# pityka/lamp

Measured on AMD Instinct MI355X. Metric: training-step samples/sec, higher is better.
Workload: dtype bf16; 1 GPU; example-cifar100 Cnn.resnet(100) training step (fwd+backprop+AdamW), synthetic CIFAR batch; per_gpu_batch=2048, global_batch=2048, parallelism=single, optimizer=AdamW lr 1e-3 wd 0 beta2 0.95 mixedPrecision

## Files before the change

include/lamp_hip.h:

```cpp
#ifndef LAMP_HIP_H
#define LAMP_HIP_H

#include <stddef.h>
#include <stdint.h>

#ifdef __cplusplus
extern "C" {
#endif

#define LAMP_MAX_DIMS 8

typedef struct lamp_tensor lamp_tensor;
typedef struct lamp_stream lamp_stream;
typedef struct lamp_comm lamp_comm;
typedef struct lamp_graph lamp_graph;

#define LAMP_U8 0
#define LAMP_I8 1
#define LAMP_I16 2
#define LAMP_I32 3
#define LAMP_I64 4
#define LAMP_F16 5
#define LAMP_F32 6
#define LAMP_F64 7
#define LAMP_BOOL 11
#define LAMP_BF16 15

#define LAMP_DEVICE_CPU (-1)

const char* lamp_last_error(void);
const char* lamp_version(void);

int lamp_has_gpu(int* out);
int lamp_get_num_gpus(int* out);
int lamp_get_device(int* out);
int lamp_set_device(int device);
int lamp_device_synchronize(void);
int lamp_flush_deferred(void);
int lamp_device_name(char* buf, int buflen);
int lamp_device_num_cus(int* out);
int lamp_stream_get_current(int device, lamp_stream** out);
int lamp_stream_get_default(int device, lamp_stream** out);
int lamp_stream_get_from_pool(int high_priority, int device, lamp_stream** out);
int lamp_stream_set_current(lamp_stream* s);
int lamp_stream_synchronize(lamp_stream* s);
int lamp_stream_wait_stream(lamp_stream* waiter, lamp_stream* on);
int lamp_stream_release(lamp_stream* s);
int lamp_tensor_record_stream(const lamp_tensor* t, lamp_stream* s_or_null);
int lamp_stream_native(lamp_stream* s, void** hip_stream_out);
int lamp_manual_seed(uint64_t seed);
int lamp_allow_tf32(int flag);

int lamp_kernel_timer_enable(int on);
// ... 529 lines not shown
```

jni/LampNative.java:

```java
package aten;

public final class LampNative {
  static { System.loadLibrary("lampjni"); }
  private LampNative() {}
  public static native String lamp_last_error();
  public static native String lamp_version();
  public static native void lamp_tensor_release_all(long[] tensors);
  public static native byte[] lamp_comm_get_unique_id();
  public static native long lamp_comm_init_rank(int nranks, byte[] id, int rank);
  public static native long[] lamp_tensors_from_file(String path, long offset, long length, boolean pin, long[] types, long[] offsets, long[] lengths);
  public static native long[] lamp_tensor_trace_list();
  public static native long[] lamp_tensor_sizes(long t);
  public static native long[] lamp_tensor_strides(long t);
  public static native boolean copyFromDoubleArray(long t, double[] a);
  public static native boolean copyToDoubleArray(long t, double[] a);
  public static native boolean copyFromFloatArray(long t, float[] a);
  public static native boolean copyToFloatArray(long t, float[] a);
  public static native boolean copyFromLongArray(long t, long[] a);
  public static native boolean copyToLongArray(long t, long[] a);
  public static native boolean copyFromIntArray(long t, int[] a);
  public static native boolean copyToIntArray(long t, int[] a);
  public static native boolean copyFromShortArray(long t, short[] a);
  public static native boolean copyToShortArray(long t, short[] a);
  public static native boolean copyFromByteArray(long t, byte[] a);
  public static native boolean copyToByteArray(long t, byte[] a);

  public static native int lamp_has_gpu();
  public static native int lamp_get_num_gpus();
  public static native int lamp_get_device();
  public static native void lamp_set_device(int device);
  public static native void lamp_device_synchronize();
  public static native void lamp_flush_deferred();
  public static native int lamp_device_num_cus();
  public static native long lamp_stream_get_current(int device);
  public static native long lamp_stream_get_default(int device);
  public static native long lamp_stream_get_from_pool(int high_priority, int device);
  public static native void lamp_stream_set_current(long s);
  public static native void lamp_stream_synchronize(long s);
  public static native void lamp_stream_wait_stream(long waiter, long on);
  public static native void lamp_stream_release(long s);
  public static native void lamp_tensor_record_stream(long t, long s_or_null);
  public static native void lamp_manual_seed(long seed);
  public static native void lamp_allow_tf32(int flag);
  public static native void lamp_kernel_timer_enable(int on);
  public static native void lamp_kernel_timer_filter(String tag);
  public static native double lamp_kernel_timer_calibrate();
  public static native void lamp_device_shared_hint(int device, int delta);
// ... 335 lines not shown
```

jni/aten_jni.c:

```c
#ifdef LAMP_JNI_SYNTAX_CHECK
#include "jni_syntax_check.h"
#else
#include <jni.h>
#endif
#include <stdint.h>
#include <stddef.h>
#include "lamp_hip.h"

#define H(x) ((void*)(intptr_t)(x))

#define LAMP_JNI_MAX_OUTS 4096

static void lamp_throw(JNIEnv* env) {
  jclass ex = (*env)->FindClass(env, "java/lang/RuntimeException");
  if (ex) (*env)->ThrowNew(env, ex, lamp_last_error());
}
static void lamp_throw_msg(JNIEnv* env, const char* msg) {
  jclass ex = (*env)->FindClass(env, "java/lang/RuntimeException");
  if (ex) (*env)->ThrowNew(env, ex, msg);
}

#define COPY_NATIVES(JT, JNAME, GET, REL)                                                                                              \
  JNIEXPORT jboolean JNICALL Java_aten_LampNative_copyFrom##JNAME##Array(JNIEnv* env, jclass cls, jlong t, JT##Array a) {              \
    (void)cls;                                                                                                                         \
// ... 120 lines not shown
  (void)cls;
  const int rc_ = lamp_set_device((int)device);
  if (rc_ != 0) { lamp_throw(env); return; }
}

JNIEXPORT void JNICALL Java_aten_LampNative_lamp_1device_1synchronize(JNIEnv* env, jclass cls) {
  (void)cls;
  const int rc_ = lamp_device_synchronize();
  if (rc_ != 0) { lamp_throw(env); return; }
}

JNIEXPORT void JNICALL Java_aten_LampNative_lamp_1flush_1deferred(JNIEnv* env, jclass cls) {
  (void)cls;
  const int rc_ = lamp_flush_deferred();
  if (rc_ != 0) { lamp_throw(env); return; }
}

JNIEXPORT jint JNICALL Java_aten_LampNative_lamp_1device_1num_1cus(JNIEnv* env, jclass cls) {
  (void)cls;
  int out_o = 0;
  const int rc_ = lamp_device_num_cus(&out_o);
  if (rc_ != 0) { lamp_throw(env); return 0; }
  return (jint)out_o;
}

JNIEXPORT jlong JNICALL Java_aten_LampNative_lamp_1stream_1get_1current(JNIEnv* env, jclass cls, jint device) {
  (void)cls;
  void* out_o = NULL;
  const int rc_ = lamp_stream_get_current((int)device, (void*)&out_o);
  if (rc_ != 0) { lamp_throw(env); return 0; }
// ... 3239 lines not shown
```

lamp_amd/csrc/core/runtime.cpp:

```cpp
#include "tensor.h"

#include <unordered_map>
#include <atomic>
#include <mutex>
#include <set>
#include <map>

struct lamp_stream {
  hipStream_t s = nullptr;
  int device = 0;
  bool is_default = false;
  std::atomic<int> refs{1};
};

struct lamp_graph {
  hipGraph_t graph = nullptr;
  hipGraphExec_t exec = nullptr;
  hipStream_t stream = nullptr;
  int device = 0;
};

namespace lamp {

namespace {
// ... 220 lines not shown
  LAMP_API_END
}
int lamp_get_device(int* out) {
  LAMP_API_BEGIN
  *out = current_device();
  LAMP_API_END
}
int lamp_set_device(int device) {
  LAMP_API_BEGIN
  set_device(device);
  LAMP_API_END
}
int lamp_flush_deferred(void) {
  LAMP_API_BEGIN
  flush_deferred();
  LAMP_API_END
}
int lamp_device_synchronize(void) {
  LAMP_API_BEGIN
  flush_deferred();
  const int dev = current_device();
  HIP_CHECK(hipDeviceSynchronize());
  check_device_asserts(dev);
  LAMP_API_END
}
int lamp_device_shared_hint(int device, int delta) {
  LAMP_API_BEGIN
  LAMP_CHECK(device >= 0 && device < 16, "device " << device << " out of range");
  device_shared_add(device, delta);
  LAMP_CHECK(device_shared(device) >= 0, "lamp_device_shared_hint: more releases than acquisitions on device " << device);
// ... 227 lines not shown
```

lamp_amd/csrc/core/switches.h:

```cpp
#pragma once
#include <cstdint>

namespace lamp {

constexpr int64_t SW_NO_CLAMP = INT64_MIN;

#define LAMP_SWITCHES_ONCE(X)                                                                                                             \
                                                        \
  X(conv_sibling, "LAMP_CONV_SIBLING", BOOL, 1, 0, "a residual block's 3x3 and its sibling 1x1 of the same input as one forward launch") \
  X(conv_chain, "LAMP_CONV_CHAIN", BOOL, 1, 0, "a convolution directly in front of a residual block and the block's 3x3 + 1x1 as one forward call (0: two)") \
  X(fuse_bn_pair, "LAMP_FUSE_BN_PAIR", BOOL, 1, 0, "relu(bn(right) + bn(left)) at a block's end as one op (0: the chain)")                \
  X(fuse_pool_logsoftmax, "LAMP_FUSE_POOL_LOGSOFTMAX", BOOL, 1, 0, "average pool -> flatten -> log-softmax tail as one node")             \
  X(fuse_block_tail, "LAMP_FUSE_BLOCK_TAIL", BOOL, 1, 0, "the last residual block and the pooled log-softmax tail as one node")          \
  X(fuse_bn_conv, "LAMP_FUSE_BN_CONV", BOOL, 1, 0, "batch norm -> relu -> convolution: the convolution applies the norm while staging")  \
  X(fuse_loss_accumulate, "LAMP_FUSE_LOSS_ACCUMULATE", BOOL, 1, 0, "acc += n * loss inside the NLL loss kernel")                          \
  X(fuse_loss_backward, "LAMP_FUSE_LOSS_BACKWARD", BOOL, 1, 0, "the NLL loss backward goes straight to the pooled log-softmax node's input in one launch")                      \
  X(fuse_loss_tail, "LAMP_FUSE_LOSS_TAIL", BOOL, 1, 0, "the loss launch also writes the pooled log-softmax's input gradient per plane")  \
  X(conv_dgrad_accumulate, "LAMP_CONV_DGRAD_ACCUMULATE", BOOL, 1, 0, "a convolution's input gradient adds into the existing one in its epilogue") \
  X(conv_dgrad_pair, "LAMP_CONV_DGRAD_PAIR", BOOL, 1, 0, "input gradients of a block's 3x3 and sibling 1x1 from one launch")             \
  X(conv_wgrad_pair, "LAMP_CONV_WGRAD_PAIR", BOOL, 1, 0, "weight gradients of a block's 3x3 and sibling 1x1 from one launch")            \
  X(conv_bwd_pair, "LAMP_CONV_BWD_PAIR", BOOL, 1, 0, "a block's paired input gradient and its two weight gradients from one call (0: the two pair calls)") \
  X(linear_bias_fused, "LAMP_LINEAR_BIAS_FUSED", BOOL, 1, 0, "a linear layer's bias in the GEMM epilogue (0: mm then add)")               \
  X(mult_add_fused, "LAMP_MULT_ADD_FUSED", BOOL, 1, 0, "x * scale + residual in one pass (0: mult then add)")                             \
  X(attention_as_written_for_cuda, "LAMP_ATTENTION_AS_WRITTEN_FOR_CUDA", BOOL, 0, 0, "multi-head attention as the reference's op chain instead of the fused kernels") \
// ... 35 lines not shown
  X(pack_cache, "LAMP_PACK_CACHE", BOOL, 1, 0, "packed filter images are cached per parameter and storage version (all four packing backends: core/pack_cache.h)") \
  X(pack_after_step, "LAMP_PACK_AFTER_STEP", BOOL, 1, 0, "the optimiser repacks every cached filter image of all four backends in place (0: lazily at first use)") \
                                                    \
  X(ig_small_d, "LAMP_IG_SMALL_D", BOOL, 1, 0, "the eight-image kernel for at most 64 output channels too")                               \
  X(ig_w8, "LAMP_IG_W8", BOOL, 1, 0, "two-image 128-row kernel: eight waves per image pair at one workgroup per CU or fewer (0: four)")  \
  X(ig_one_image, "LAMP_IG_ONE_IMAGE", BOOL, 1, 0, "... one image per workgroup at one image per CU or fewer (0: pairs)")                 \
                                                                                                 \
  X(wgrad_group, "LAMP_WGRAD_GROUP", BOOL, 1, 0, "two layers' eight-wave weight gradients parked and launched as one (0: every layer at once)") \
  X(wgrad_min_ips, "LAMP_WGRAD_MIN_IPS", INT, 0, 2, "fewest images per weight-gradient workgroup; unset (0): 2 up to 512 images, 8 above") \
  X(wg8h_dma, "LAMP_WG8H_DMA", BOOL, 1, 0, "eight-wave weight-gradient kernel: dY tiles by LDS-DMA (0: through registers, the bitwise reference of the DMA's hand-counted waits)") \
  X(defer_wgrad_reduce, "LAMP_DEFER_WGRAD_REDUCE", BOOL, 1, 0, "weight-gradient partial sums are reduced in batches, deferred until someone reads them")

#define LAMP_SWITCHES_PER_CALL(X)                                                                                                         \
  X(ig_variant, "LAMP_IG_VARIANT", LETTER, 0, 0, "bf16 implicit GEMM kernel form: b two-image 128-row, d eight-image at any batch; unset or any other letter: by geometry") \
  X(ig_ktail, "LAMP_IG_KTAIL", BOOL, 1, 0, "a 3x3's 1 .. 8 channels beyond the last whole K chunk from their own packed image (0: the padded chunk)") \
  X(knn_split_dbg, "LAMP_KNN_SPLIT_DBG", INT, 0, SW_NO_CLAMP, "3: the k-NN filter's kernel counts visits, candidates and selection cycles per wave and prints them")

using SwType_BOOL = bool;
using SwType_INT = int64_t;
using SwType_LETTER = char;
#define LAMP_SWITCH_MEMBER(member, name, kind, dflt, lo, doc) SwType_##kind member;
struct Switches { LAMP_SWITCHES_ONCE(LAMP_SWITCH_MEMBER) };
struct SwitchesNow { LAMP_SWITCHES_PER_CALL(LAMP_SWITCH_MEMBER) };
#undef LAMP_SWITCH_MEMBER

const Switches& sw();
SwitchesNow sw_now();

}
```

lamp_amd/csrc/core/tensor.h:

```cpp
#pragma once
#include <hip/hip_runtime.h>
#include <atomic>
#include <cstdint>
#include <cstring>
#include <stdexcept>
#include <string>
#include <vector>
#include <sstream>

#include "../../../include/lamp_hip.h"

namespace lamp {

constexpr int kMaxDims = LAMP_MAX_DIMS;

enum DType : int {
  kU8 = 0, kI8 = 1, kI16 = 2, kI32 = 3, kI64 = 4, kF16 = 5, kF32 = 6, kF64 = 7, kBool = 11, kBF16 = 15
};

inline size_t dtype_size(int dt) {
  switch (dt) {
    case kU8: case kI8: case kBool: return 1;
    case kI16: case kF16: case kBF16: return 2;
    case kI32: case kF32: return 4;
// ... 63 lines not shown
  bool owned = true;
  void* pool = nullptr;
  void* map_base = nullptr;
  size_t map_len = 0;
  size_t pinned_capacity = 0;
  std::atomic<int> refs{1};
  std::atomic<uint64_t> version{0};
  uint64_t uid = next_uid();
  static uint64_t next_uid() { static std::atomic<uint64_t> c{1}; return c.fetch_add(1, std::memory_order_relaxed); }
  std::atomic<uint32_t> pending{0};
  std::atomic<uint32_t> deferred_reads{0};
  bool scratch = false;
};
void resolve_deferred(Storage* st);
void flush_deferred();

}

struct lamp_tensor {
  lamp::Storage* st = nullptr;
  int64_t offset = 0;
  int ndim = 0;
  int64_t sizes[lamp::kMaxDims] = {0};
  int64_t strides[lamp::kMaxDims] = {0};
  int dtype = lamp::kF32;

  int64_t numel() const {
    int64_t n = 1;
    for (int i = 0; i < ndim; i++) n *= sizes[i];
    return n;
// ... 130 lines not shown
```

lamp_amd/csrc/kernels/norm.hip:

```cpp
#include "device_utils.h"
#include <atomic>
#include <map>
#include <mutex>
#include <type_traits>
#include "../core/strided.h"
#include "../core/switches.h"

namespace lamp {

template <class A> struct Welford {
  A n, mean, m2;
};
template <class A> __device__ __forceinline__ void wf_add(Welford<A>& w, A x) {
  w.n += A(1);
  A d = x - w.mean;
  w.mean += d / w.n;
  w.m2 += d * (x - w.mean);
}
template <class A> __device__ __forceinline__ Welford<A> wf_merge(const Welford<A>& a, const Welford<A>& b) {
  Welford<A> r;
  r.n = a.n + b.n;
  if (r.n == A(0)) { r.mean = 0; r.m2 = 0; return r; }
  A d = b.mean - a.mean;
  A f = b.n / r.n;
// ... 273 lines not shown
      if (adsrc) {
        T a = adsrc[base];
        if (second.x) a = store_as<T>(bn_affine<A>(load_as<A>(a), mu2, scale2, bb2));
        o = store_as<T>((A)(load_as<A>(o) + load_as<A>(a)));
      }
      if (relu && load_as<A>(o) < A(0)) o = store_as<T>(A(0));
      y[base] = o;
    }
  }
}

template <class T>
__global__ __launch_bounds__(256) void bn_bwd_reduce_kernel(const T* __restrict__ dy, const T* __restrict__ x, const T* __restrict__ mean,
                                                            acc_t<T>* __restrict__ partial, int64_t N, int64_t C, int64_t HW, int nsplit, int vec,
                                                            int relu, const T* __restrict__ invstd, const T* __restrict__ w, const T* __restrict__ b,
                                                            const T* __restrict__ addend) {
  using A = acc_t<T>;
  constexpr int W = 16 / sizeof(T);
  __shared__ A sm[2][4];
  const int64_t c = blockIdx.x;
  const int split = blockIdx.y;
  const A mu = load_as<A>(mean[c]);
  const A scale = relu ? load_as<A>(invstd[c]) * (w ? load_as<A>(w[c]) : A(1)) : A(0);
  const A bb = (relu && b) ? load_as<A>(b[c]) : A(0);
  A s1 = 0, s2 = 0;
  if (vec) {
    const int64_t vpp = HW / W, total = N * vpp;
    for (int64_t i = (int64_t)split * blockDim.x + threadIdx.x; i < total; i += (int64_t)nsplit * blockDim.x) {
      const int64_t n = i / vpp, v = i - n * vpp;
      const int64_t base = (n * C + c) * HW + v * W;
      const Vec<T, W> g = *reinterpret_cast<const Vec<T, W>*>(dy + base);
      const Vec<T, W> xv = *reinterpret_cast<const Vec<T, W>*>(x + base);
      Vec<T, W> ad;
// ... 116 lines not shown
      const A gm = sums[c * 2] * (A)inv_m;
      r = (g - gm - (xx - mu) * k) * is * wc;
    } else {
      r = g * is * wc;
    }
    dx[i] = store_as<T>(r);
  }
}

template <class T>
__global__ __launch_bounds__(256) void bn_bwd_apply2_kernel(const T* __restrict__ dy, const T* __restrict__ x, const T* __restrict__ mean,
                                                            const T* __restrict__ invstd, const T* __restrict__ w, const T* __restrict__ b,
                                                            const acc_t<T>* __restrict__ partial, int nsplit, T* dweight, T* dbias,
                                                            T* __restrict__ dx, int64_t N, int64_t C, int64_t HW, int nblk, double inv_m,
                                                            int training, int vec, int relu, int do_apply, const T* __restrict__ addend,
                                                            T* __restrict__ dadd) {
  using A = acc_t<T>;
  constexpr int W = 16 / sizeof(T);
  __shared__ A stat[2];
  const int64_t c = blockIdx.x;
  const int slice = blockIdx.y;
  const A is = load_as<A>(invstd[c]);
  if (threadIdx.x < 64) {
    const int lane = threadIdx.x;
    A a = 0, bs = 0;
    for (int s = lane; s < nsplit; s += 64) { a += partial[((int64_t)s * C + c) * 2]; bs += partial[((int64_t)s * C + c) * 2 + 1]; }
    a = wave_sum(a); bs = wave_sum(bs);
    if (lane == 0) {
      stat[0] = a; stat[1] = bs;
      if (slice == 0) {
        if (dweight) dweight[c] = store_as<T>((A)(bs * is));
        if (dbias) dbias[c] = store_as<T>(a);
      }
// ... 128 lines not shown
  static __device__ __forceinline__ void zero_if(uint4& p, int q, bool off) { (&p.x)[q >> 1] &= !off ? ~0u : (q & 1) ? 0x0000ffffu : 0xffff0000u; }
  static __device__ __forceinline__ void put(uint4& p, int q, float v) {
    unsigned& w = (&p.x)[q >> 1];
    const unsigned b = bf16_t(v).bits;
    w = (q & 1) ? (w | (b << 16)) : b;
  }
  static __device__ __forceinline__ float centred(float g, float gm, float x, float mu, float kk) { return __builtin_fmaf(-(x - mu), kk, g - gm); }
};

template <class T> struct BnFusedDual { const T* mean2; const T* invstd2; const T* w2; const T* b2; T* dweight2; T* dbias2; };
template <class T, int NP, bool RELU, bool ADD, bool DUAL, bool PLANES>
__global__ __launch_bounds__(512, NP <= 2 ? 8 : 2) void bn_bwd_fused_kernel(const T* __restrict__ dy, const T* __restrict__ x, const T* __restrict__ mean, const T* __restrict__ invstd,
                                                           const T* __restrict__ w, const T* __restrict__ b, unsigned long long* slots, unsigned long long* slots2,
                                                           unsigned* depart, T* dweight, T* dbias, T* __restrict__ dx, int64_t N, int C, int HW, int S, double inv_m,
                                                           const T* __restrict__ addend, T* __restrict__ dadd, int vshift, int* assert_word, int c0,
                                                           BnFusedDual<T> dual, int dy_sc) {
  static_assert(!(DUAL || PLANES) || std::is_same<T, bf16_t>::value, "the dual and plane forms exist in bf16");
  using P = BnPacket<T>;
  using A = typename P::A;
  constexpr int W = P::W;
  constexpr int NS = DUAL ? 3 : 2;
  __shared__ A sm[NS][8];
  __shared__ A stat[NS];
  const int cl = blockIdx.x / S, s = blockIdx.x - cl * S, c = c0 + cl;
  const int tid = threadIdx.x, lane = tid & 63, wid = tid >> 6;
  const int vpp = HW >> (W == 8 ? 3 : W == 4 ? 2 : 1);
  const int64_t total = N * vpp;
  const A mu = load_as<A>(mean[c]), is = load_as<A>(invstd[c]);
  const A wc = w ? load_as<A>(w[c]) : A(1);
  const A scale = is * wc, bb = (RELU && b) ? load_as<A>(b[c]) : A(0);
  const A mu2 = DUAL ? load_as<A>(dual.mean2[c]) : A(0), is2 = DUAL ? load_as<A>(dual.invstd2[c]) : A(0);
// ... 415 lines not shown
  for (int b = 0; b < 31; b++) if (vpp == ((int64_t)1 << b)) return b;
  return -1;
}
template <class T>
static const void* bn_fused_kernel_for(int NP, bool relu, bool add, bool dual, bool planes) {
#define BN_FUSED_K(NPv, R, AD, D, P) ((const void*)bn_bwd_fused_kernel<T, NPv, R, AD, D, P>)
#define BN_FUSED_NP(R, AD, D, P) (NP == 1 ? BN_FUSED_K(1, R, AD, D, P) : NP == 2 ? BN_FUSED_K(2, R, AD, D, P) : NP == 4 ? BN_FUSED_K(4, R, AD, D, P) \
                                  : NP == 8 ? BN_FUSED_K(8, R, AD, D, P) : BN_FUSED_K(16, R, AD, D, P))
  if constexpr (std::is_same<T, bf16_t>::value) {
    if (dual) return planes ? BN_FUSED_NP(true, true, true, true) : BN_FUSED_NP(true, true, true, false);
  }
  return add ? BN_FUSED_NP(true, true, false, false) : relu ? BN_FUSED_NP(true, false, false, false) : BN_FUSED_NP(false, false, false, false);
#undef BN_FUSED_NP
#undef BN_FUSED_K
}
struct BnPlaneGrad { const bf16_t* p = nullptr; int sn = 0, sc = 0; };
template <class T>
static bool bn_bwd_fused_launch(const Tensor* gc, const Tensor* xc, const Tensor* mean_t, const Tensor* invstd_t, const Tensor* weight, const Tensor* bias,
                                Tensor* dw, Tensor* db, Tensor* dx, Tensor* dadd, const Tensor* addc, const BnGeom& g, int relu, hipStream_t st,
                                const BnDualHost* dualh = nullptr, BnPlaneGrad gplanes = BnPlaneGrad()) {
  constexpr bool BF16 = std::is_same<T, bf16_t>::value;
  constexpr int W = 16 / (int)sizeof(T);
  if (!bn_fused_gate(xc->device(), !BF16) || g.HW % W != 0) return false;
  const int64_t packets = g.N * (g.HW / W);
  if (packets <= 0 || packets >= (int64_t)1 << 30 || xc->numel() / W >= (int64_t)1 << 31) return false;
  if (addc && !relu) return false;
  const bool planes = gplanes.p != nullptr;
  if (planes && !(dualh && g.HW == 64 && gplanes.sn == 1 && g.N % 8 == 0 && gplanes.sc % 8 == 0 && ((uintptr_t)gplanes.p & 15) == 0)) return false;
  const int cus = num_cus();
  const int np_mask = (int)sw().bn_fused_np_mask;
// ... 10 lines not shown
      if (g.C * sl.s <= resident(k)) { kfn = k; S = sl.s; }
    }
    if (!kfn) return false;
  } else {
    const BnFusedSlices sl = bn_fused_slices(packets, g.C, cus, 1);
    if (!(np_mask & sl.NP)) return false;
    kfn = bn_fused_kernel_for<T>(sl.NP, relu, addc, false, false);
    const int64_t r = resident(kfn);
    if (sl.s > r) return false;
    S = sl.s;
    chunk = std::min<int64_t>(std::min<int64_t>(g.C, r / S), BN_FUSED_MAXC);
  }
  BnFusedSync sync = bn_fused_sync_state(xc->device(), st);
  if (!sync.depart) return false;
  const double passes = (dx ? 3.0 : 2.0) + (addc ? 1.0 : 0.0) + (dadd ? 1.0 : 0.0) - (planes ? 1.0 : 0.0);
  KernelTimer kt("bn_bwd_fused", 0, passes * (double)xc->numel() * sizeof(T), st);
  auto in = [](const Tensor* t) { return t ? t->ptr<T>() : (const T*)nullptr; };
  auto out = [](Tensor* t) { return t ? t->ptr<T>() : (T*)nullptr; };
  const T* dyp = in(gc); const T* xp = in(xc); const T* mp = in(mean_t); const T* ip = in(invstd_t); const T* wp = in(weight); const T* bp = in(bias);
  const T* adp = in(addc);
  T* dwp = out(dw); T* dbp = out(db); T* dxp = out(dx); T* dap = out(dadd);
  BnFusedDual<T> dual{};
  int a_sc = 0;
  if constexpr (BF16) {
    if (planes) { dyp = gplanes.p; a_sc = gplanes.sc; }
    if (dualh) dual = BnFusedDual<T>{in(dualh->mean2), in(dualh->invstd2), in(dualh->w2), in(dualh->b2), out(dualh->dw2), out(dualh->db2)};
  }
  int64_t a_N = g.N; int a_C = (int)g.C, a_HW = (int)g.HW, a_S = (int)S;
  double inv_m = 1.0 / (double)(g.N * g.HW);
  int a_vshift = bn_fused_vshift(g.HW / W);
  int* awp = device_assert_word(xc->device());
  for (int64_t c0 = 0; c0 < g.C; c0 += chunk) {
    int a_c0 = (int)c0;
    const int64_t nc = std::min<int64_t>(chunk, g.C - c0);
    void* args[] = {(void*)&dyp, (void*)&xp, (void*)&mp, (void*)&ip, (void*)&wp, (void*)&bp, (void*)&sync.slots, (void*)&sync.slots2, (void*)&sync.depart, (void*)&dwp,
                    (void*)&dbp, (void*)&dxp, (void*)&a_N, (void*)&a_C, (void*)&a_HW, (void*)&a_S, (void*)&inv_m, (void*)&adp, (void*)&dap, (void*)&a_vshift, (void*)&awp,
                    (void*)&a_c0, (void*)&dual, (void*)&a_sc};
    HIP_CHECK(hipLaunchKernel(kfn, dim3((unsigned)(nc * S)), dim3(512), args, 0, st));
  }
  return true;
}
static BnPlaneGrad plane_broadcast_base(const Tensor* g) {
  BnPlaneGrad r;
  if (!g || g->dtype != kBF16 || g->ndim != 4 || !g->is_device()) return r;
  if (g->sizes[2] * g->sizes[3] <= 1 || g->strides[2] != 0 || g->strides[3] != 0) return r;
  const int64_t sn = g->sizes[0] > 1 ? g->strides[0] : 0, sc = g->sizes[1] > 1 ? g->strides[1] : 0;
  if (sn < 0 || sc < 0 || sn >= ((int64_t)1 << 24) || sc >= ((int64_t)1 << 24) || (g->sizes[0] - 1) * sn + (g->sizes[1] - 1) * sc >= ((int64_t)1 << 31)) return r;
  r.p = g->ptr<bf16_t>(); r.sn = (int)sn; r.sc = (int)sc;
  return r;
}
static void check_cvec(const Tensor* t, int64_t C, int dtype, const char* what) {
  if (!t) return;
  check_device_tensor(t, what);
// ... 223 lines not shown
    using A = acc_t<T>;
    const int vec = (g.HW % (16 / sizeof(T)) == 0) && (((uintptr_t)X->data() | (uintptr_t)G->data() | (uintptr_t)(dx.get() ? dx->data() : nullptr) |
                                                          (uintptr_t)(AD ? AD->data() : nullptr) | (uintptr_t)(dadd.get() ? dadd->data() : nullptr)) & 15) == 0;
    const bool col = g.HW < 64;
    bool fused_done = false;
    if constexpr (!std::is_same<T, f16_t>::value) {
      if (training && vec && !col && total > 0 && (dx.get() || dadd.get()))
        fused_done = bn_bwd_fused_launch<T>(G, X, mean_t, invstd_t, weight, bias, dw.get(), db.get(), dx.get(), dadd.get(), AD, g, relu, st);
    }
    if (!fused_done) {
    const int64_t blocks = col ? (g.C + 255) / 256 : g.C;
    const int nsplit = pick_split(blocks, g.N);
    int64_t ps[1] = {(int64_t)nsplit * g.C * 2};
    int64_t ss[1] = {g.C * 2};
    Hold partial(new_tensor(ps, 1, acc_dtype<A>(), x->device())), sums(new_tensor(ss, 1, acc_dtype<A>(), x->device()));
    {
      KernelTimer kt1("bn_bwd_reduce", 0, 2.0 * (double)total * sizeof(T), st);
      if (col) hipLaunchKernelGGL((bn_bwd_reduce_col_kernel<T>), dim3((unsigned)blocks, nsplit), dim3(256), 0, st, G->ptr<T>(), X->ptr<T>(), mean_t->ptr<T>(), partial->ptr<A>(), g.N, g.C, g.HW, nsplit);
      else hipLaunchKernelGGL((bn_bwd_reduce_kernel<T>), dim3((unsigned)g.C, nsplit), dim3(256), 0, st, G->ptr<T>(), X->ptr<T>(), mean_t->ptr<T>(), partial->ptr<A>(), g.N, g.C, g.HW, nsplit, vec,
                              relu, invstd_t->ptr<T>(), weight ? weight->ptr<T>() : (const T*)nullptr, bias ? bias->ptr<T>() : (const T*)nullptr,
                              AD ? AD->ptr<T>() : (const T*)nullptr);
    }
    LAMP_LAUNCH_CHECK();
    T* dwp = dw.get() ? dw->ptr<T>() : (T*)nullptr;
    T* dbp = db.get() ? db->ptr<T>() : (T*)nullptr;
    const T* wp = weight ? weight->ptr<T>() : (const T*)nullptr;
    const T* bp = bias ? bias->ptr<T>() : (const T*)nullptr;
    if (!col) {
      const int do_apply = ((dx.get() || dadd.get()) && total > 0) ? 1 : 0;
      const int nblk = do_apply ? nsplit : 1;
      KernelTimer kt2("bn_bwd_apply", 0, 3.0 * (double)total * sizeof(T), st);
      hipLaunchKernelGGL((bn_bwd_apply2_kernel<T>), dim3((unsigned)g.C, nblk), dim3(256), 0, st, G->ptr<T>(), X->ptr<T>(), mean_t->ptr<T>(), invstd_t->ptr<T>(),
                         wp, bp, partial->ptr<A>(), nsplit, dwp, dbp, dx.get() ? dx->ptr<T>() : (T*)nullptr, g.N, g.C, g.HW, nblk,
                         1.0 / (double)(g.N * g.HW), training, vec, relu, do_apply, AD ? AD->ptr<T>() : (const T*)nullptr,
                         dadd.get() ? dadd->ptr<T>() : (T*)nullptr);
      LAMP_LAUNCH_CHECK();
    } else {
      hipLaunchKernelGGL((bn_bwd_finalize_kernel<T>), dim3((unsigned)((g.C * 64 + 255) / 256)), dim3(256), 0, st, partial->ptr<A>(), sums->ptr<A>(), g.C,
                         nsplit, invstd_t->ptr<T>(), dwp, dbp);
      LAMP_LAUNCH_CHECK();
      if (dx.get() && total > 0) {
        KernelTimer kt2("bn_bwd_apply", 0, 3.0 * (double)total * sizeof(T), st);
        hipLaunchKernelGGL((bn_bwd_apply_kernel<T>), dim3(grid_for(total, 256)), dim3(256), 0, st, G->ptr<T>(), X->ptr<T>(), mean_t->ptr<T>(),
                           invstd_t->ptr<T>(), wp, sums->ptr<A>(), dx->ptr<T>(), total, g.C, g.HW, 1.0 / (double)(g.N * g.HW), training, vec, relu, bp);
        LAMP_LAUNCH_CHECK();
      }
    }
    }
  });
  out3[0] = dx.take(); out3[1] = dw.take(); out3[2] = db.take();
// ... 232 lines not shown
```

lamp_amd/csrc/kernels/wgrad_reduce.h:

```cpp
#pragma once
#include <vector>
#include "conv_geom.h"
#include "device_utils.h"

namespace lamp {

struct WgradReduceArgs {
  int kind;
  const float* partial;
  void* dw;
  int dw_f32;
  int CO, CI, CIP, COP, RS;
  int nsplit;
  int O;
  int blocks;
  int cached;
};

__device__ __forceinline__ void wgrad_reduce_igemm(const WgradReduceArgs& a, int block, float4 (*red)[32]) {
  const int M = a.COP;
  const int q = threadIdx.x & 31, sg = threadIdx.x >> 5;
  const int per_split = a.RS * M * a.CIP / 4;
  const int col = block * 32 + q;
  float4 s = make_float4(0.f, 0.f, 0.f, 0.f);
  const int c4 = a.CIP / 4;
  const int row = col / c4;
  const int ci = (col - row * c4) * 4, rs = row / M, co = row - rs * M;
  const bool real = col < per_split && co < a.CO && ci < a.CI;
  if (real) {
    const float4* p4 = reinterpret_cast<const float4*>(a.partial) + col;
#pragma unroll 4
    for (int sp = sg; sp < a.nsplit; sp += 8) {
      typedef float nt_f4 __attribute__((ext_vector_type(4)));
      float4 v;
      if (a.cached) v = p4[(int64_t)sp * per_split];
      else { const nt_f4 nv = __builtin_nontemporal_load(reinterpret_cast<const nt_f4*>(&p4[(int64_t)sp * per_split])); v = make_float4(nv[0], nv[1], nv[2], nv[3]); }
      s.x += v.x; s.y += v.y; s.z += v.z; s.w += v.w;
    }
  }
  red[sg][q] = s;
  __syncthreads();
  if (sg == 0 && real) {
#pragma unroll
// ... 6 lines not shown
        if (a.dw_f32) static_cast<float*>(a.dw)[o] = r[k]; else static_cast<bf16_t*>(a.dw)[o] = bf16_t(r[k]);
      }
  }
}

__device__ __forceinline__ void wgrad_reduce_narrow(const WgradReduceArgs& a, int block) {
  const int lane = threadIdx.x & 63;
  const int o = (int)(((int64_t)block * 256 + threadIdx.x) >> 6);
  if (o >= a.O) return;
  float s = 0.f;
  for (int b = lane; b < a.nsplit; b += 64) s += a.partial[(int64_t)b * a.O + o];
  s = wave_sum(s);
  if (lane == 0) { if (a.dw_f32) static_cast<float*>(a.dw)[o] = s; else static_cast<bf16_t*>(a.dw)[o] = bf16_t(s); }
}

void wgrad_reduce_enqueue(const WgradReduceArgs& a, lamp_tensor* partial, lamp_tensor* dw, hipStream_t st);
bool wgrad_reduce_deferred();
struct Wg8hProblem { const lamp_tensor* dy; const lamp_tensor* x; lamp_tensor* dw; ConvGeom g; const lamp_tensor* affine; };
void wgrad_park(const Wg8hProblem& p, hipStream_t st);
struct WgradReduction { WgradReduceArgs a; Hold partial, dw; };
struct SecondWgradConv;
void wg8h_launch(const Wg8hProblem& a, const Wg8hProblem* b, hipStream_t st, const SecondWgradConv* second, std::vector<WgradReduction>* out);

}
```

lamp_amd/csrc/kernels/wgrad_reduce.hip:

```cpp
#include "wgrad_reduce.h"
#include "../core/switches.h"
#include <algorithm>
#include <mutex>
#include <thread>
#include <vector>

namespace lamp {

constexpr int WR_MAX = 16;
struct WgradReduceMany { WgradReduceArgs e[WR_MAX]; };

__global__ __launch_bounds__(256) void wgrad_reduce_many_kernel(WgradReduceMany m) {
  __shared__ float4 red[8][32];
  const WgradReduceArgs& a = m.e[blockIdx.y];
  if ((int)blockIdx.x >= a.blocks) return;
  if (a.kind == 0) wgrad_reduce_igemm(a, blockIdx.x, red);
  else wgrad_reduce_narrow(a, blockIdx.x);
}

namespace {
struct Entry { Wg8hProblem p; WgradReduceArgs a; Tensor* partial; hipStream_t st; int device; std::thread::id owner; };
std::mutex g_mu;
std::vector<Entry> g_list;

void count_reads(const Wg8hProblem& p, uint32_t d) {
  for (const Tensor* t : {p.dy, p.x, p.affine}) if (t) t->st->deferred_reads.fetch_add(d, std::memory_order_acq_rel);
}
bool names(const Entry& e, const Storage* st) {
  return e.p.dw->st == st || (e.p.dy && (e.p.dy->st == st || e.p.x->st == st || (e.p.affine && e.p.affine->st == st)));
}
struct Taken {
// ... 3 lines not shown
    for (auto& e : v) for (const Tensor* t : {e.p.dy, e.p.x, e.p.affine, (const Tensor*)e.p.dw, (const Tensor*)e.partial}) release(const_cast<Tensor*>(t));
  }
};
void wg8h_launch_locked(const Entry e, const Wg8hProblem* b, std::vector<Entry>& into) {
  const int prev = current_device();
  if (prev != e.device) set_device(e.device);
  struct Back { int prev, dev; ~Back() { if (prev != dev) set_device(prev); } } back{prev, e.device};
  std::vector<WgradReduction> out;
  wg8h_launch(e.p, b, e.st, nullptr, &out);
  for (auto& r : out) {
    if (e.st != current_stream(e.device)) record_stream(r.partial.get(), e.device, e.st);
    into.push_back(Entry{Wg8hProblem{nullptr, nullptr, r.dw.get(), {}, nullptr}, r.a, r.partial.get(), e.st, e.device, e.owner});
    r.dw->st->pending.fetch_add(1, std::memory_order_release);
    r.dw.take(); r.partial.take();
  }
}

void launch_batch(const std::vector<Entry>& v) {
  std::vector<bool> done(v.size(), false);
  for (size_t i = 0; i < v.size(); i++) {
    if (done[i] || !v[i].partial) continue;
    WgradReduceMany m;
    int cnt = 0, maxb = 0;
    for (size_t j = i; j < v.size() && cnt < WR_MAX; j++) {
      if (done[j] || !v[j].partial || v[j].st != v[i].st || v[j].device != v[i].device) continue;
      m.e[cnt] = v[j].a;
      m.e[cnt].partial = reinterpret_cast<const float*>(static_cast<const char*>(v[j].partial->st->ptr)) + v[j].partial->offset;
      m.e[cnt].dw = static_cast<char*>(v[j].p.dw->st->ptr) + v[j].p.dw->offset * (v[j].a.dw_f32 ? 4 : 2);
      v[j].p.dw->st->version.fetch_add(1, std::memory_order_relaxed);
      maxb = std::max(maxb, v[j].a.blocks);
// ... 58 lines not shown
    return e.p.dy && e.owner == me && e.st == st && e.device == dev && e.p.g.N == p.g.N && e.p.dw->st != p.dw->st;
  });
  if (m != g_list.end()) {
    Taken t{{*m}};
    g_list.erase(m);
    wg8h_launch_locked(t.v[0], &p, g_list);
    return;
  }
  Entry e{Wg8hProblem{retain(p.dy), retain(p.x), retain(p.dw), p.g, p.affine ? retain(p.affine) : nullptr}, {}, nullptr, st, dev, me};
  g_list.push_back(e);
  count_reads(e.p, 1);
  p.dw->st->version.fetch_add(1, std::memory_order_relaxed);
  p.dw->st->pending.fetch_add(1, std::memory_order_release);
}

bool wgrad_reduce_deferred() {
  const bool defer = sw().defer_wgrad_reduce;
  return defer;
}
void wgrad_reduce_enqueue(const WgradReduceArgs& a, lamp_tensor* partial, lamp_tensor* dw, hipStream_t st) {
  const bool defer = wgrad_reduce_deferred();
  if (!defer || !dw->st->owned) {
    WgradReduceMany m;
    m.e[0] = a;
    m.e[0].cached = defer ? 0 : 1;
    m.e[0].partial = partial->ptr<float>();
    m.e[0].dw = dw->data();
    hipLaunchKernelGGL(wgrad_reduce_many_kernel, dim3((unsigned)a.blocks, 1), dim3(256), 0, st, m);
    LAMP_LAUNCH_CHECK();
    return;
// ... 9 lines not shown
```

Baseline: 2.269 million samples/s.

## Run pending weight-gradient reductions as extra workgroups of bf16 batch-norm backward launches

After: 2.287 million samples/s, median of 6. No clear change (+0.8%).

```diff
diff --git a/include/lamp_hip.h b/include/lamp_hip.h
--- a/include/lamp_hip.h
+++ b/include/lamp_hip.h
@@ -37,6 +37,7 @@
 int lamp_set_device(int device);
 int lamp_device_synchronize(void);
 int lamp_flush_deferred(void);
+int lamp_deferred_pending(int* out);
 int lamp_device_name(char* buf, int buflen);
 int lamp_device_num_cus(int* out);
 int lamp_stream_get_current(int device, lamp_stream** out);
diff --git a/jni/LampNative.java b/jni/LampNative.java
--- a/jni/LampNative.java
+++ b/jni/LampNative.java
@@ -31,6 +31,7 @@
   public static native void lamp_set_device(int device);
   public static native void lamp_device_synchronize();
   public static native void lamp_flush_deferred();
+  public static native int lamp_deferred_pending();
   public static native int lamp_device_num_cus();
   public static native long lamp_stream_get_current(int device);
   public static native long lamp_stream_get_default(int device);
diff --git a/jni/aten_jni.c b/jni/aten_jni.c
--- a/jni/aten_jni.c
+++ b/jni/aten_jni.c
@@ -158,6 +158,14 @@
   (void)cls;
   const int rc_ = lamp_flush_deferred();
   if (rc_ != 0) { lamp_throw(env); return; }
+}
+
+JNIEXPORT jint JNICALL Java_aten_LampNative_lamp_1deferred_1pending(JNIEnv* env, jclass cls) {
+  (void)cls;
+  int out_o = 0;
+  const int rc_ = lamp_deferred_pending(&out_o);
+  if (rc_ != 0) { lamp_throw(env); return 0; }
+  return (jint)out_o;
 }
 
 JNIEXPORT jint JNICALL Java_aten_LampNative_lamp_1device_1num_1cus(JNIEnv* env, jclass cls) {
diff --git a/lamp_amd/csrc/core/runtime.cpp b/lamp_amd/csrc/core/runtime.cpp
--- a/lamp_amd/csrc/core/runtime.cpp
+++ b/lamp_amd/csrc/core/runtime.cpp
@@ -258,6 +258,12 @@
 int lamp_flush_deferred(void) {
   LAMP_API_BEGIN
   flush_deferred();
+  LAMP_API_END
+}
+int lamp_deferred_pending(int* out) {
+  LAMP_API_BEGIN
+  LAMP_CHECK(out != nullptr, "out is null");
+  *out = deferred_pending();
   LAMP_API_END
 }
 int lamp_device_synchronize(void) {
diff --git a/lamp_amd/csrc/core/switches.h b/lamp_amd/csrc/core/switches.h
--- a/lamp_amd/csrc/core/switches.h
+++ b/lamp_amd/csrc/core/switches.h
@@ -73,6 +73,10 @@
 #define LAMP_SWITCHES_PER_CALL(X)                                                                                                         \
   X(ig_variant, "LAMP_IG_VARIANT", LETTER, 0, 0, "bf16 implicit GEMM kernel form: b two-image 128-row, d eight-image at any batch; unset or any other letter: by geometry") \
   X(ig_ktail, "LAMP_IG_KTAIL", BOOL, 1, 0, "a 3x3's 1 .. 8 channels beyond the last whole K chunk from their own packed image (0: the padded chunk)") \
+  X(wgrad_reduce_ride, "LAMP_WGRAD_REDUCE_RIDE", BOOL, 1, 0, "pending weight-gradient reductions ride as extra workgroups of the small bf16 batch-norm backward launches (0: all in the batch at the end of backprop)") \
+  X(wgrad_ride_k, "LAMP_WGRAD_RIDE_K", INT, 2, 0, "... a host takes riders of at most this many times its own declared bytes (0: no limit)") \
+  X(wgrad_ride_host_bytes, "LAMP_WGRAD_RIDE_HOST_BYTES", INT, 8 << 20, 0, "... hosts are batch-norm backward launches on activations of at most this many bytes") \
+  X(wgrad_ride_budget, "LAMP_WGRAD_RIDE_BUDGET", INT, -1, SW_NO_CLAMP, "... debug: every host's rider budget in bytes instead of the rule (negative: the rule)") \
   X(knn_split_dbg, "LAMP_KNN_SPLIT_DBG", INT, 0, SW_NO_CLAMP, "3: the k-NN filter's kernel counts visits, candidates and selection cycles per wave and prints them")
 
 using SwType_BOOL = bool;
diff --git a/lamp_amd/csrc/core/tensor.h b/lamp_amd/csrc/core/tensor.h
--- a/lamp_amd/csrc/core/tensor.h
+++ b/lamp_amd/csrc/core/tensor.h
@@ -101,6 +101,7 @@
 };
 void resolve_deferred(Storage* st);
 void flush_deferred();
+int deferred_pending();
 
 }
 
diff --git a/lamp_amd/csrc/kernels/norm.hip b/lamp_amd/csrc/kernels/norm.hip
--- a/lamp_amd/csrc/kernels/norm.hip
+++ b/lamp_amd/csrc/kernels/norm.hip
@@ -5,6 +5,7 @@
 #include <type_traits>
 #include "../core/strided.h"
 #include "../core/switches.h"
+#include "wgrad_reduce.h"
 
 namespace lamp {
 
@@ -311,9 +312,17 @@
 __global__ __launch_bounds__(256) void bn_bwd_reduce_kernel(const T* __restrict__ dy, const T* __restrict__ x, const T* __restrict__ mean,
                                                             acc_t<T>* __restrict__ partial, int64_t N, int64_t C, int64_t HW, int nsplit, int vec,
                                                             int relu, const T* __restrict__ invstd, const T* __restrict__ w, const T* __restrict__ b,
-                                                            const T* __restrict__ addend) {
+                                                            const T* __restrict__ addend, const WgradRiders riders) {
   using A = acc_t<T>;
   constexpr int W = 16 / sizeof(T);
+  if constexpr (std::is_same<T, bf16_t>::value) {
+    kernargs_now(dy, x, mean, partial, N, C, HW, nsplit, vec, relu, invstd, w, b, addend);
+    if ((int)blockIdx.x >= riders.host) {
+      __shared__ float4 red[1][8][32];
+      wgrad_ride<1>(riders, (int)(blockIdx.y * (gridDim.x - riders.host) + blockIdx.x - riders.host), red);
+      return;
+    }
+  }
   __shared__ A sm[2][4];
   const int64_t c = blockIdx.x;
   const int split = blockIdx.y;
@@ -460,9 +469,17 @@
                                                             const acc_t<T>* __restrict__ partial, int nsplit, T* dweight, T* dbias,
                                                             T* __restrict__ dx, int64_t N, int64_t C, int64_t HW, int nblk, double inv_m,
                                                             int training, int vec, int relu, int do_apply, const T* __restrict__ addend,
-                                                            T* __restrict__ dadd) {
+                                                            T* __restrict__ dadd, const WgradRiders riders) {
   using A = acc_t<T>;
   constexpr int W = 16 / sizeof(T);
+  if constexpr (std::is_same<T, bf16_t>::value) {
+    kernargs_now(dy, x, mean, invstd, w, b, partial, nsplit, dx, N, C, HW, nblk, training, vec, relu, do_apply, addend, dadd);
+    if ((int)blockIdx.x >= riders.host) {
+      __shared__ float4 red[1][8][32];
+      wgrad_ride<1>(riders, (int)(blockIdx.y * (gridDim.x - riders.host) + blockIdx.x - riders.host), red);
+      return;
+    }
+  }
   __shared__ A stat[2];
   const int64_t c = blockIdx.x;
   const int slice = blockIdx.y;
@@ -621,7 +638,15 @@
                                                            const T* __restrict__ w, const T* __restrict__ b, unsigned long long* slots, unsigned long long* slots2,
                                                            unsigned* depart, T* dweight, T* dbias, T* __restrict__ dx, int64_t N, int C, int HW, int S, double inv_m,
                                                            const T* __restrict__ addend, T* __restrict__ dadd, int vshift, int* assert_word, int c0,
-                                                           BnFusedDual<T> dual, int dy_sc) {
+                                                           BnFusedDual<T> dual, int dy_sc, const WgradRiders riders) {
+  if constexpr (std::is_same<T, bf16_t>::value) {
+    kernargs_now(dy, x, mean, invstd, w, b, dx, N, C, HW, S, addend, dadd, vshift, c0);
+    if ((int)blockIdx.x >= riders.host) {
+      __shared__ float4 red[2][8][32];
+      wgrad_ride<2>(riders, (int)blockIdx.x - riders.host, red);
+      return;
+    }
+  }
   static_assert(!(DUAL || PLANES) || std::is_same<T, bf16_t>::value, "the dual and plane forms exist in bf16");
   using P = BnPacket<T>;
   using A = typename P::A;
@@ -1067,6 +1092,13 @@
 #undef BN_FUSED_NP
 #undef BN_FUSED_K
 }
+static double wgrad_ride_budget(bool bf16, double act_bytes, double host_bytes) {
+  if (!bf16) return 0;
+  const SwitchesNow s = sw_now();
+  if (!s.wgrad_reduce_ride || act_bytes > (double)s.wgrad_ride_host_bytes) return 0;
+  if (s.wgrad_ride_budget >= 0) return (double)s.wgrad_ride_budget;
+  return s.wgrad_ride_k > 0 ? (double)s.wgrad_ride_k * host_bytes : 1e30;
+}
 struct BnPlaneGrad { const bf16_t* p = nullptr; int sn = 0, sc = 0; };
 template <class T>
 static bool bn_bwd_fused_launch(const Tensor* gc, const Tensor* xc, const Tensor* mean_t, const Tensor* invstd_t, const Tensor* weight, const Tensor* bias,
@@ -1107,8 +1139,7 @@
   BnFusedSync sync = bn_fused_sync_state(xc->device(), st);
   if (!sync.depart) return false;
   const double passes = (dx ? 3.0 : 2.0) + (addc ? 1.0 : 0.0) + (dadd ? 1.0 : 0.0) - (planes ? 1.0 : 0.0);
-  KernelTimer kt("bn_bwd_fused", 0, passes * (double)xc->numel() * sizeof(T), st);
-  auto in = [](const Tensor* t) { return t ? t->ptr<T>() : (const T*)nullptr; };
+  auto in =[](const Tensor* t) { return t ? t->ptr<T>() : (const T*)nullptr; };
   auto out = [](Tensor* t) { return t ? t->ptr<T>() : (T*)nullptr; };
   const T* dyp = in(gc); const T* xp = in(xc); const T* mp = in(mean_t); const T* ip = in(invstd_t); const T* wp = in(weight); const T* bp = in(bias);
   const T* adp = in(addc);
@@ -1123,13 +1154,19 @@
   double inv_m = 1.0 / (double)(g.N * g.HW);
   int a_vshift = bn_fused_vshift(g.HW / W);
   int* awp = device_assert_word(xc->device());
+  const double act_bytes = (double)xc->numel() * sizeof(T), host_bytes = passes * act_bytes;
+  WgradRide ride(xc->device(), st, wgrad_ride_budget(BF16 && chunk == g.C, act_bytes, host_bytes));
+  KernelTimer kt("bn_bwd_fused", 0, host_bytes + ride.bytes, st);
+  WgradRiders riders = ride.r;
+  const int rider_wgs = (ride.blocks() + 1) / 2;
   for (int64_t c0 = 0; c0 < g.C; c0 += chunk) {
     int a_c0 = (int)c0;
     const int64_t nc = std::min<int64_t>(chunk, g.C - c0);
+    riders.host = (int)(nc * S);
     void* args[] = {(void*)&dyp, (void*)&xp, (void*)&mp, (void*)&ip, (void*)&wp, (void*)&bp, (void*)&sync.slots, (void*)&sync.slots2, (void*)&sync.depart, (void*)&dwp,
                     (void*)&dbp, (void*)&dxp, (void*)&a_N, (void*)&a_C, (void*)&a_HW, (void*)&a_S, (void*)&inv_m, (void*)&adp, (void*)&dap, (void*)&a_vshift, (void*)&awp,
-                    (void*)&a_c0, (void*)&dual, (void*)&a_sc};
-    HIP_CHECK(hipLaunchKernel(kfn, dim3((unsigned)(nc * S)), dim3(512), args, 0, st));
+                    (void*)&a_c0, (void*)&dual, (void*)&a_sc, (void*)&riders};
+    HIP_CHECK(hipLaunchKernel(kfn, dim3((unsigned)(nc * S + rider_wgs)), dim3(512), args, 0, st));
   }
   return true;
 }
@@ -1383,26 +1420,38 @@
     int64_t ps[1] = {(int64_t)nsplit * g.C * 2};
     int64_t ss[1] = {g.C * 2};
     Hold partial(new_tensor(ps, 1, acc_dtype<A>(), x->device())), sums(new_tensor(ss, 1, acc_dtype<A>(), x->device()));
-    {
-      KernelTimer kt1("bn_bwd_reduce", 0, 2.0 * (double)total * sizeof(T), st);
-      if (col) hipLaunchKernelGGL((bn_bwd_reduce_col_kernel<T>), dim3((unsigned)blocks, nsplit), dim3(256), 0, st, G->ptr<T>(), X->ptr<T>(), mean_t->ptr<T>(), partial->ptr<A>(), g.N, g.C, g.HW, nsplit);
-      else hipLaunchKernelGGL((bn_bwd_reduce_kernel<T>), dim3((unsigned)g.C, nsplit), dim3(256), 0, st, G->ptr<T>(), X->ptr<T>(), mean_t->ptr<T>(), partial->ptr<A>(), g.N, g.C, g.HW, nsplit, vec,
-                              relu, invstd_t->ptr<T>(), weight ? weight->ptr<T>() : (const T*)nullptr, bias ? bias->ptr<T>() : (const T*)nullptr,
-                              AD ? AD->ptr<T>() : (const T*)nullptr);
-    }
-    LAMP_LAUNCH_CHECK();
+    const T* Gp = G->ptr<T>(); const T* Xp = X->ptr<T>(); const T* ADp = AD ? AD->ptr<T>() : (const T*)nullptr;
+    const T* mp = mean_t->ptr<T>(); const T* ip = invstd_t->ptr<T>();
+    A* pp = partial->ptr<A>();
     T* dwp = dw.get() ? dw->ptr<T>() : (T*)nullptr;
     T* dbp = db.get() ? db->ptr<T>() : (T*)nullptr;
+    T* dxp = dx.get() ? dx->ptr<T>() : (T*)nullptr;
+    T* dap = dadd.get() ? dadd->ptr<T>() : (T*)nullptr;
     const T* wp = weight ? weight->ptr<T>() : (const T*)nullptr;
     const T* bp = bias ? bias->ptr<T>() : (const T*)nullptr;
+    constexpr bool BF16 = std::is_same<T, bf16_t>::value;
+    const double act_bytes = (double)total * sizeof(T);
+    auto rider_columns = [](const WgradRide& ride, int ny) { return (unsigned)((ride.blocks() + ny - 1) / ny); };
+    if (col) {
+      KernelTimer kt1("bn_bwd_reduce", 0, 2.0 * act_bytes, st);
+      hipLaunchKernelGGL((bn_bwd_reduce_col_kernel<T>), dim3((unsigned)blocks, nsplit), dim3(256), 0, st, Gp, Xp, mp, pp, g.N, g.C, g.HW, nsplit);
+    } else {
+      WgradRide ride(x->device(), st, wgrad_ride_budget(BF16, act_bytes, 2.0 * act_bytes));
+      KernelTimer kt1("bn_bwd_reduce", 0, 2.0 * act_bytes + ride.bytes, st);
+      ride.r.host = (int)g.C;
+      hipLaunchKernelGGL((bn_bwd_reduce_kernel<T>), dim3((unsigned)g.C + rider_columns(ride, nsplit), nsplit), dim3(256), 0, st, Gp, Xp, mp, pp, g.N, g.C, g.HW, nsplit, vec,
+                         relu, ip, wp, bp, ADp, ride.r);
+    }
+    LAMP_LAUNCH_CHECK();
     if (!col) {
       const int do_apply = ((dx.get() || dadd.get()) && total > 0) ? 1 : 0;
       const int nblk = do_apply ? nsplit : 1;
-      KernelTimer kt2("bn_bwd_apply", 0, 3.0 * (double)total * sizeof(T), st);
-      hipLaunchKernelGGL((bn_bwd_apply2_kernel<T>), dim3((unsigned)g.C, nblk), dim3(256), 0, st, G->ptr<T>(), X->ptr<T>(), mean_t->ptr<T>(), invstd_t->ptr<T>(),
-                         wp, bp, partial->ptr<A>(), nsplit, dwp, dbp, dx.get() ? dx->ptr<T>() : (T*)nullptr, g.N, g.C, g.HW, nblk,
-                         1.0 / (double)(g.N * g.HW), training, vec, relu, do_apply, AD ? AD->ptr<T>() : (const T*)nullptr,
-                         dadd.get() ? dadd->ptr<T>() : (T*)nullptr);
+      WgradRide ride(x->device(), st, do_apply ? wgrad_ride_budget(BF16, act_bytes, 3.0 * act_bytes) : 0.0);
+      KernelTimer kt2("bn_bwd_apply", 0, 3.0 * act_bytes + ride.bytes, st);
+      ride.r.host = (int)g.C;
+      hipLaunchKernelGGL((bn_bwd_apply2_kernel<T>), dim3((unsigned)g.C + rider_columns(ride, nblk), nblk), dim3(256), 0, st, Gp, Xp, mp, ip,
+                         wp, bp, pp, nsplit, dwp, dbp, dxp, g.N, g.C, g.HW, nblk,
+                         1.0 / (double)(g.N * g.HW), training, vec, relu, do_apply, ADp, dap, ride.r);
       LAMP_LAUNCH_CHECK();
     } else {
       hipLaunchKernelGGL((bn_bwd_finalize_kernel<T>), dim3((unsigned)((g.C * 64 + 255) / 256)), dim3(256), 0, st, partial->ptr<A>(), sums->ptr<A>(), g.C,
diff --git a/lamp_amd/csrc/kernels/wgrad_reduce.h b/lamp_amd/csrc/kernels/wgrad_reduce.h
--- a/lamp_amd/csrc/kernels/wgrad_reduce.h
+++ b/lamp_amd/csrc/kernels/wgrad_reduce.h
@@ -17,16 +17,16 @@
   int cached;
 };
 
-__device__ __forceinline__ void wgrad_reduce_igemm(const WgradReduceArgs& a, int block, float4 (*red)[32]) {
+__device__ __forceinline__ void wgrad_reduce_igemm(const WgradReduceArgs& a, int block, float4 (*red)[32], int tid, bool live = true) {
   const int M = a.COP;
-  const int q = threadIdx.x & 31, sg = threadIdx.x >> 5;
+  const int q = tid & 31, sg = tid >> 5;
   const int per_split = a.RS * M * a.CIP / 4;
   const int col = block * 32 + q;
   float4 s = make_float4(0.f, 0.f, 0.f, 0.f);
   const int c4 = a.CIP / 4;
   const int row = col / c4;
   const int ci = (col - row * c4) * 4, rs = row / M, co = row - rs * M;
-  const bool real = col < per_split && co < a.CO && ci < a.CI;
+  const bool real = live && col < per_split && co < a.CO && ci < a.CI;
   if (real) {
     const float4* p4 = reinterpret_cast<const float4*>(a.partial) + col;
 #pragma unroll 4
@@ -63,6 +63,32 @@
   if (lane == 0) { if (a.dw_f32) static_cast<float*>(a.dw)[o] = s; else static_cast<bf16_t*>(a.dw)[o] = bf16_t(s); }
 }
 
+constexpr int WR_MAX = 16;
+constexpr int WR_RIDE_MAX = 16;
+struct WgradRiders { WgradReduceArgs e[WR_RIDE_MAX]; int first[WR_RIDE_MAX + 1]; int n; int host; };
+template <class A> __device__ __forceinline__ void sgpr_now(A a) { asm volatile("" ::"s"(a)); }
+template <class... A> __device__ __forceinline__ void kernargs_now(A... a) { (sgpr_now(a), ...); }
+template <int TEAMS>
+__device__ __forceinline__ void wgrad_ride(const WgradRiders& r, int wg, float4 (*red)[8][32]) {
+  const int team = TEAMS > 1 ? __builtin_amdgcn_readfirstlane((int)threadIdx.x >> 8) : 0;
+  const int f = wg * TEAMS + team;
+  const bool live = f < r.first[r.n];
+  if (TEAMS == 1 && !live) return;
+  int j = 0;
+  while (j + 1 < r.n && f >= r.first[j + 1]) j++;
+  wgrad_reduce_igemm(r.e[j], f - r.first[j], red[team], (int)threadIdx.x & 255, live);
+}
+struct WgradRide {
+  WgradRide(int device, hipStream_t st, double budget_bytes);
+  ~WgradRide();
+  WgradRide(const WgradRide&) = delete;
+  WgradRide& operator=(const WgradRide&) = delete;
+  WgradRiders r;
+  double bytes = 0;
+  int blocks() const { return r.first[r.n]; }
+  void* held = nullptr;
+};
+
 void wgrad_reduce_enqueue(const WgradReduceArgs& a, lamp_tensor* partial, lamp_tensor* dw, hipStream_t st);
 bool wgrad_reduce_deferred();
 struct Wg8hProblem { const lamp_tensor* dy; const lamp_tensor* x; lamp_tensor* dw; ConvGeom g; const lamp_tensor* affine; };
diff --git a/lamp_amd/csrc/kernels/wgrad_reduce.hip b/lamp_amd/csrc/kernels/wgrad_reduce.hip
--- a/lamp_amd/csrc/kernels/wgrad_reduce.hip
+++ b/lamp_amd/csrc/kernels/wgrad_reduce.hip
@@ -7,14 +7,13 @@
 
 namespace lamp {
 
-constexpr int WR_MAX = 16;
 struct WgradReduceMany { WgradReduceArgs e[WR_MAX]; };
 
 __global__ __launch_bounds__(256) void wgrad_reduce_many_kernel(WgradReduceMany m) {
   __shared__ float4 red[8][32];
   const WgradReduceArgs& a = m.e[blockIdx.y];
   if ((int)blockIdx.x >= a.blocks) return;
-  if (a.kind == 0) wgrad_reduce_igemm(a, blockIdx.x, red);
+  if (a.kind == 0) wgrad_reduce_igemm(a, blockIdx.x, red, threadIdx.x);
   else wgrad_reduce_narrow(a, blockIdx.x);
 }
 
@@ -48,6 +47,10 @@
     r.dw->st->pending.fetch_add(1, std::memory_order_release);
     r.dw.take(); r.partial.take();
   }
+}
+
+double reduction_bytes(const WgradReduceArgs& a) {
+  return (double)a.nsplit * a.RS * a.COP * a.CIP * 4.0 + (double)a.CO * a.CI * a.RS * (a.dw_f32 ? 4.0 : 2.0);
 }
 
 void launch_batch(const std::vector<Entry>& v) {
@@ -136,6 +139,48 @@
   p.dw->st->pending.fetch_add(1, std::memory_order_release);
 }
 
+namespace { struct RideHeld { std::unique_lock<std::mutex> lk; Taken t; }; }
+WgradRide::WgradRide(int device, hipStream_t st, double budget_bytes) {
+  r.n = 0; r.first[0] = 0; r.host = 0;
+  if (!(budget_bytes > 0)) return;
+  const std::thread::id me = std::this_thread::get_id();
+  auto* h = new RideHeld{std::unique_lock<std::mutex>(g_mu), {}};
+  size_t keep = 0;
+  bool open = true;
+  for (size_t i = 0; i < g_list.size(); i++) {
+    const Entry& e = g_list[i];
+    bool take = false;
+    if (open && e.partial && e.a.kind == 0 && e.owner == me && e.device == device && e.st == st) {
+      const double b = reduction_bytes(e.a);
+      take = r.n < WR_RIDE_MAX && bytes + b <= budget_bytes && (int64_t)r.first[r.n] + e.a.blocks < ((int64_t)1 << 30);
+      if (take) {
+        WgradReduceArgs& a = r.e[r.n];
+        a = e.a;
+        a.partial = reinterpret_cast<const float*>(static_cast<const char*>(e.partial->st->ptr)) + e.partial->offset;
+        a.dw = static_cast<char*>(e.p.dw->st->ptr) + e.p.dw->offset * (e.a.dw_f32 ? 4 : 2);
+        e.p.dw->st->version.fetch_add(1, std::memory_order_relaxed);
+        r.first[r.n + 1] = r.first[r.n] + e.a.blocks;
+        r.n++;
+        bytes += b;
+        h->t.v.push_back(e);
+      } else open = false;
+    }
+    if (!take) g_list[keep++] = g_list[i];
+  }
+  g_list.resize(keep);
+  if (r.n == 0) delete h; else held = h;
+}
+WgradRide::~WgradRide() {
+  if (!held) return;
+  auto* h = static_cast<RideHeld*>(held);
+  { Taken done; done.v.swap(h->t.v); }
+  delete h;
+}
+int deferred_pending() {
+  std::lock_guard<std::mutex> lk(g_mu);
+  return (int)g_list.size();
+}
+
 bool wgrad_reduce_deferred() {
   const bool defer = sw().defer_wgrad_reduce;
   return defer;
```
